# Polochon-street/bliss-rs

Measured on AMD Instinct MI355X. Metric: songs/sec (3-min 22 050 Hz f32) at 1/2/4/8 GPU; HBM GB/s vs roofline, higher is better.
Workload: dtype f32; 1 GPU; configs[1]: batch of 1024 synthetic 3969000-sample (3-min) white-noise f32 PCM buffers per GPU, full 23-feature descriptor set (FeaturesVersion 2); songs_per_gpu=1024, songs_total=1024, features=23, parallelism=single GPU

## Files before the change

bliss-rs_amd/csrc/ctx.hpp:

```cpp
#pragma once
#include <hip/hip_runtime.h>
#include <sched.h>

#include <map>
#include <memory>
#include <mutex>
#include <string>
#include <vector>

#include "../../include/blissgpu.h"
#include "internal.hpp"
#include "resample.hpp"
#include "staging_ring.hpp"

namespace bg {

int fail(int code, const char* what, const char* detail);

#define HIP_TRY(expr)                                                                           \
    do {                                                                                        \
        hipError_t e_ = (expr);                                                                 \
        if (e_ != hipSuccess) return ::bg::fail(BLISSGPU_ERR_HIP, #expr, hipGetErrorString(e_)); \
    } while (0)

struct EventPair { hipEvent_t a, b; };

template <typename T>
struct DevBuf {
    T* p = nullptr;
    size_t cap = 0;
    int ensure(size_t n) {
        if (n <= cap) return BLISSGPU_OK;
        if (p) (void)hipFree(p);
        p = nullptr;
        cap = 0;
        size_t want = n + n / 8 + 64;
        hipError_t e = hipMalloc((void**)&p, want * sizeof(T));
        if (e != hipSuccess && want > n) {
            (void)hipGetLastError();
            want = n;
            e = hipMalloc((void**)&p, want * sizeof(T));
        }
        if (e != hipSuccess) {
            (void)hipGetLastError();
            p = nullptr;
            return fail(BLISSGPU_ERR_OOM, "hipMalloc", hipGetErrorString(e));
        }
        cap = want;
        return BLISSGPU_OK;
    }
    void release() { if (p) (void)hipFree(p); p = nullptr; cap = 0; }
};

template <typename T>
struct PinnedBuf {
    T* p = nullptr;
    size_t cap = 0;
    int ensure(size_t n) {
        if (n <= cap) return BLISSGPU_OK;
        if (p) (void)hipHostFree(p);
        p = nullptr;
        cap = 0;
        const size_t want = n + n / 4 + 64;
        hipError_t e = hipHostMalloc((void**)&p, want * sizeof(T), hipHostMallocDefault);
        if (e != hipSuccess) { (void)hipGetLastError(); p = nullptr; return fail(BLISSGPU_ERR_OOM, "hipHostMalloc", hipGetErrorString(e)); }
        cap = want;
        return BLISSGPU_OK;
    }
    void release() { if (p) (void)hipHostFree(p); p = nullptr; cap = 0; }
};

struct ChunkSlot {
    DevBuf<uint8_t> slab;
    DevBuf<uint8_t> desc;
    PinnedBuf<uint8_t> h_desc;
    hipEvent_t ev_start = nullptr, ev_fork = nullptr, ev_stft = nullptr, ev_sel = nullptr, ev_tune = nullptr, ev_sum = nullptr, ev_chroma = nullptr;
    hipEvent_t ev_acf = nullptr, ev_beat = nullptr;
    bool beat_masked = false;
    static constexpr int MAX_PIECES = 8;
    hipEvent_t ev_piece[MAX_PIECES] = {};
    int pieces = 0;
    bg::SongRange piece[MAX_PIECES]{};
    hipEvent_t ev_desc = nullptr;
    hipEvent_t ev_free = nullptr;
    bool used = false;
    bool back_pending = false;
    Batch batch{};
    Workspace ws{};
};

#ifndef FEED_COPY_STREAMS
#define FEED_COPY_STREAMS 2
#endif
#ifndef STAGE_LANES_DEFAULT
#define STAGE_LANES_DEFAULT 4
#endif
#ifndef STAGE_SLABS_DEFAULT
#define STAGE_SLABS_DEFAULT 3
#endif
#ifndef STAGE_SLAB_KIB_DEFAULT
#define STAGE_SLAB_KIB_DEFAULT 4096
#endif
#ifndef STAGE_EVENT_FLAGS
#define STAGE_EVENT_FLAGS (hipEventDisableTiming | hipEventBlockingSync)
#endif
constexpr int N_COPY_STREAMS = FEED_COPY_STREAMS;
#ifndef FEED_BUFFERS
#define FEED_BUFFERS 3
#endif
constexpr int N_FEED_BUFFERS = FEED_BUFFERS;
constexpr uint32_t MAX_SAMPLE_RATE = 768000;
struct FeedSong {
    const void* p;
    uint64_t frames;
    uint32_t rate;
    uint8_t fmt;
    uint8_t channels;
    size_t frame_bytes() const { return (size_t)(fmt == BLISSGPU_SAMPLE_S16 ? 2 : 4) * channels; }
    bool direct() const { return fmt == BLISSGPU_SAMPLE_F32 && channels == 1 && rate == SWR_OUT_RATE; }
};
struct ResampleBank {
    SwrPlan plan;
    float* d_bank = nullptr;
    size_t bytes = 0;
    uint64_t last_use = 0;
};
#ifndef SWR_CACHE_BYTES
#define SWR_CACHE_BYTES (64ull << 20)
#endif

constexpr int MAX_STAGE_LANES = 16;
struct HipStageDev {
    int device;
    hipStream_t* streams;
    std::vector<int> cpus;
    void thread_begin(int) {
        (void)hipSetDevice(device);
        if (!cpus.empty()) {
            cpu_set_t set;
            CPU_ZERO(&set);
            for (int cpu : cpus)
                if (cpu >= 0 && cpu < CPU_SETSIZE) CPU_SET(cpu, &set);
            (void)sched_setaffinity(0, sizeof(set), &set);
        }
    }
    void* slab_alloc(size_t bytes) {
        void* p = nullptr;
        if (hipHostMalloc(&p, bytes, hipHostMallocDefault) != hipSuccess) { (void)hipGetLastError(); return nullptr; }
        return p;
    }
    void slab_free(void* p) { (void)hipHostFree(p); }
    void* event_create() {
        hipEvent_t e = nullptr;
        if (hipEventCreateWithFlags(&e, STAGE_EVENT_FLAGS) != hipSuccess) { (void)hipGetLastError(); return nullptr; }
        return (void*)e;
    }
    void event_destroy(void* e) { (void)hipEventDestroy((hipEvent_t)e); }
    int copy_async(void* dst, const void* slab, size_t bytes, int lane) {
        return (int)hipMemcpyAsync(dst, slab, bytes, hipMemcpyHostToDevice, streams[lane]);
    }
    int event_record(void* ev, int lane) { return (int)hipEventRecord((hipEvent_t)ev, streams[lane]); }
    int event_wait(void* ev) { return (int)hipEventSynchronize((hipEvent_t)ev); }
    std::string error_string(int code) { return hipGetErrorString((hipError_t)code); }
};

struct HostFeed {
    DevBuf<float> pcm[N_FEED_BUFFERS];
    DevBuf<uint8_t> raw[N_FEED_BUFFERS];
    DevBuf<float> out[N_FEED_BUFFERS];
    hipEvent_t ev_copied[N_FEED_BUFFERS][N_COPY_STREAMS] = {}, ev_done[N_FEED_BUFFERS] = {};
    hipStream_t copy_stream[N_COPY_STREAMS] = {};
    StageConfig stage_cfg{STAGE_LANES_DEFAULT, STAGE_SLABS_DEFAULT, (size_t)STAGE_SLAB_KIB_DEFAULT << 10};
    std::unique_ptr<StagingRing<HipStageDev>> ring;
    hipStream_t lane_stream[MAX_STAGE_LANES] = {};
    hipEvent_t ev_lane[N_FEED_BUFFERS][MAX_STAGE_LANES] = {};
    bool stage_numa = false;
    bool stage_numa_known = false;
    uint64_t staged_calls = 0;
    uint64_t staged_bytes = 0;
};

}

struct blissgpu_ctx {
    int device = 0;
    std::recursive_mutex mu;
    hipStream_t own_stream = nullptr;
    hipStream_t stream = nullptr;
    hipStream_t aux_stream = nullptr;
    hipStream_t chr_stream = nullptr;
    hipStream_t mask_stream = nullptr;
    int mask_cus = 0;
    int tail_mode = -1;
    uint32_t pipeline_chunks = 1;
    hipEvent_t ev_interop = nullptr;
    bool rolloff_exact_all = false;
    bool flux_order = false;
    int stft_shape = 0;
    int tail_split = 0;
    bool debug_chroma = false;
    bool serial = false;
    bool counted_live = false;
    uint64_t ws_limit = 0;
    uint32_t cand_budget = bg::CAND_BUDGET_PER_FRAME;
    float2 *tw8192 = nullptr, *tw512 = nullptr;
    float *hann8192 = nullptr, *hannz512 = nullptr, *bt_rwv = nullptr, *bt_dfwv = nullptr;
    double* chroma_bank = nullptr;
    bg::DeviceTables tables{};
    bg::ChunkSlot slot[2];
    uint64_t chunk_seq = 0;
    bg::DevBuf<int32_t> dbg_tuning;
    bg::DevBuf<uint32_t> dbg_nbpms;
    bg::DevBuf<double> dbg_chroma, dbg_interval;
    uint32_t dbg_n = 0;
    bg::Workspace last_ws{};
    std::vector<bg::SongDesc> last_songs;
    uint64_t last_chunks = 0;
    bg::HostFeed feed;
    std::map<uint32_t, bg::ResampleBank> swr_banks;
    size_t swr_bytes = 0;
    uint64_t swr_clock = 0;
    int64_t forest_split = 0;
    bool forest_global = false;
    int64_t forest_group_nodes = 0;
    bg::DevBuf<uint32_t> gf_img[2];
    bg::PinnedBuf<uint32_t> gf_host[2];
    hipEvent_t gf_ev[2] = {nullptr, nullptr};
    double gf_build_ms = 0.0, gf_wait_ms = 0.0;
    uint64_t gf_batches = 0;
    int n_cus = 0;
    bg::DevBuf<uint32_t> pl_sync, pl_keys;
    bg::DevBuf<uint32_t> pl_next;
    bg::DevBuf<uint8_t> pl_tmp;
    bg::DevBuf<unsigned long long> pl_slots;
    bg::DevBuf<uint8_t> pl_chain;
    bg::DevBuf<uint8_t> km_ws;
    uint64_t km_loop_copies = 0, km_loop_bytes = 0;
// ... 76 lines not shown
```

bliss-rs_amd/csrc/kernels_tempo.hip:

```cpp
#include "device_utils.hpp"
#include "internal.hpp"

namespace bg {

__device__ __forceinline__ float exp_f32(float x) { return (float)exp((double)x); }

__global__ __launch_bounds__(256) void onset_kernel(const SongDesc* __restrict__ songs,
                                                    const float* __restrict__ flux,
                                                    float* __restrict__ thresholded) {
    const SongDesc sd = songs[blockIdx.y];
    const uint32_t t = blockIdx.x * 256 + threadIdx.x;
    if (!sd.ok || t >= sd.n_b) return;
    const float* f = flux + sd.b_off;
    float p[7], tmp[7];
#pragma unroll
    for (int i = 0; i < 7; i++) {
        const long idx = (long)t - 6 + i;
        p[i] = idx >= 0 ? f[idx] : 0.0f;
    }
    const float b0 = 0.1599879f, b1 = 0.31997577f, b2 = 0.1599879f, a1 = 0.23484048f, a2 = 0.0f;
    float x1 = 0.f, x2 = 0.f, y1 = 0.f, y2 = 0.f;
#pragma unroll
    for (int i = 0; i < 7; i++) {
        const float x0 = p[i];
        const float y0 = b0 * x0 + b1 * x1 + b2 * x2 - a1 * y1 - a2 * y2;
        x2 = x1; x1 = x0; y2 = y1; y1 = y0;
        p[i] = y0;
    }
#pragma unroll
    for (int i = 0; i < 7; i++) tmp[6 - i] = p[i];
    x1 = x2 = y1 = y2 = 0.f;
#pragma unroll
    for (int i = 0; i < 7; i++) {
        const float x0 = tmp[i];
        const float y0 = b0 * x0 + b1 * x1 + b2 * x2 - a1 * y1 - a2 * y2;
        x2 = x1; x1 = x0; y2 = y1; y1 = y0;
        tmp[i] = y0;
    }
#pragma unroll
    for (int i = 0; i < 7; i++) p[i] = tmp[6 - i];
    float sum = 0.0f;
#pragma unroll
    for (int i = 0; i < 7; i++) sum += p[i];
    const float mean = sum / 7.0f;
    const float p5 = p[5];
#pragma unroll
    for (int i = 0; i < 7; i++)
#pragma unroll
        for (int j = 0; j + 1 < 7 - i; j++) {
            const float lo = fminf(p[j], p[j + 1]), hi = fmaxf(p[j], p[j + 1]);
            p[j] = lo; p[j + 1] = hi;
        }
    const float median = p[3];
    thresholded[sd.b_off + t] = p5 - median - mean * 0.3f;
}

void launch_onset(const Batch& b, const Workspace& w, hipStream_t st) {
    if (b.n_songs == 0 || b.total_b == 0) return;
    hipLaunchKernelGGL(onset_kernel, dim3((uint32_t)((b.max_nb + 255) / 256), b.n_songs), dim3(256), 0, st, b.songs,
                       w.flux, w.thresholded);
}

template <int Q>
__device__ __forceinline__ void wave_argmax_last(const float (&x)[Q], float* val, int* idx) {
    const int lane = lane_id();
    float best = -1.0f;
    int bidx = 0;
#pragma unroll
    for (int q = 0; q < Q; q++) {
        if (x[q] >= 0.0f && x[q] >= best) { best = x[q]; bidx = lane + 64 * q; }
    }
#pragma unroll
    for (int off = 32; off > 0; off >>= 1) {
        const float ov = __shfl_xor(best, off, WAVE);
        const int oi = __shfl_xor(bidx, off, WAVE);
        if (ov > best || (ov == best && oi > bidx)) { best = ov; bidx = oi; }
    }
    *val = best;
    *idx = (best < 0.0f) ? 0 : bidx;
}

__device__ __forceinline__ float quad_peak_pos(const float* x, int len, int pos) {
    if (pos == 0 || pos >= len - 1) return (float)pos;
    const float s0 = x[pos - 1], s1 = x[pos], s2 = x[pos + 1];
    return (float)pos + 0.5f * (s0 - s2) / (s0 - 2.0f * s1 + s2);
}

__device__ float bt_timesig(const float* acf, long gp) {
    if (gp < 2) return 4;
    float three = 0.0f, four = 0.0f;
    const long acflen = BT_WINLEN;
    if (acflen > 6 * gp + 2) {
        for (long k = -2; k < 2; k++) { three += acf[3 * gp + k]; four += acf[4 * gp + k]; }
    } else {
        for (long k = -2; k < 2; k++) {
            const long i3 = 3 * gp + k, i6 = 6 * gp + k, i4 = 4 * gp + k, i2 = 2 * gp + k;
            if (i3 < acflen && i6 < acflen) three += acf[i3] + acf[i6];
            else if (i3 < acflen) three += acf[i3];
            if (i4 < acflen && i2 < acflen) four += acf[i4] + acf[i2];
            else if (i4 < acflen) four += acf[i4];
        }
    }
    return three > four ? 3 : 4;
}

constexpr int BT_PRE_G3 = 0, BT_PRE_G4 = BT_LAGLEN, BT_PRE_RP3 = 256, BT_PRE_RP4 = 257, BT_PRE_TS3 = 258, BT_PRE_TS4 = 259;
static_assert(BT_PRE_STRIDE >= 260, "per-run record");

typedef float bt_f2 __attribute__((ext_vector_type(2)));

constexpr int ACF_RUNS = 8, ACF_PITCH = 580;
static_assert(ACF_PITCH >= BT_WINLEN + 65 && ACF_PITCH % 4 == 0, "zero padding behind a frame, 16-byte aligned frames");

__device__ __forceinline__ void acf_block16(bt_f2 (&acc)[4], const float* w, const float* w1, const float* f) {
    float r[24], r1[24], fv[16];
#pragma unroll
    for (int u = 0; u < 24; u++) { r[u] = w[u]; r1[u] = w1[u]; }
#pragma unroll
    for (int u = 0; u < 16; u++) fv[u] = f[u];
#pragma unroll
    for (int u = 0; u < 16; u += 2) {
        const bt_f2 fv0 = {fv[u], fv[u]}, fv1 = {fv[u + 1], fv[u + 1]};
#pragma unroll
        for (int k = 0; k < 4; k++) {
            const bt_f2 e = {r[u + 2 * k], r[u + 2 * k + 1]};
            acc[k] = acc[k] + fv0 * e;
        }
#pragma unroll
        for (int k = 0; k < 4; k++) {
            const bt_f2 o = {r1[u + 2 * k], r1[u + 2 * k + 1]};
            acc[k] = acc[k] + fv1 * o;
        }
    }
}

__global__ __launch_bounds__(256) void beat_acf_kernel(const SongDesc* __restrict__ songs,
                                                       const float* __restrict__ thresholded,
                                                       const float* __restrict__ rwv_tab,
                                                       float* __restrict__ pre_all) {
    __shared__ __attribute__((aligned(16))) float df[ACF_RUNS * ACF_PITCH];
    __shared__ __attribute__((aligned(16))) float df1[ACF_RUNS * ACF_PITCH];
    static_assert(ACF_PITCH >= BT_WINLEN && ACF_PITCH >= 2 * BT_LAGLEN, "acf / acfout live in a run's own frame");
    const uint32_t s = blockIdx.y;
    const long m0 = (long)blockIdx.x * ACF_RUNS;
    const SongDesc sd = songs[s];
    if (!sd.ok) return;
    const long n_b = sd.n_b;
    const long n_runs = (n_b >= BT_STEP) ? (n_b - BT_STEP) / BT_STEP + 1 : 0;
    if (m0 >= n_runs) return;
    const int tid = threadIdx.x, lane = tid & 63;
    const int wave = __builtin_amdgcn_readfirstlane(tid >> 6);
    const float* thr = thresholded + sd.b_off;

    {
        constexpr int per = ACF_RUNS * ACF_PITCH / 256 + 1;
        float v[per];
#pragma unroll
        for (int q = 0; q < per; q++) {
            const int e = tid + 256 * q, r = e / ACF_PITCH, i = e - r * ACF_PITCH;
            const long m = m0 + r, xi = 128 * (m + 1) - 512 + i;
            const bool live = e < ACF_RUNS * ACF_PITCH && i < BT_WINLEN && m < n_runs && xi > 0;
            const float x = thr[live ? xi - 1 : 0];
            v[q] = live ? x : 0.0f;
        }
#pragma unroll
        for (int q = 0; q < per; q++) {
            const int e = tid + 256 * q, r = e / ACF_PITCH, i = e - r * ACF_PITCH;
            if (e < ACF_RUNS * ACF_PITCH) {
                df[e] = v[q];
                if (i > 0) df1[e - 1] = v[q];
                if (i == ACF_PITCH - 1) df1[e] = 0.0f;
            }
        }
    }
    __syncthreads();
    const int r = lane >> 3, g = lane & 7;
    const int la = 64 * wave + 8 * g, lb = BT_WINLEN - 8 - 64 * wave - 8 * g;
    bt_f2 sa[4], sb[4];
    {
        const int na = BT_WINLEN - 64 * wave, nb = 64 * (wave + 1);
        const float* fr = df + r * ACF_PITCH;
        const float* fr1 = df1 + r * ACF_PITCH;
#pragma unroll
        for (int k = 0; k < 4; k++) { sa[k] = bt_f2{0.0f, 0.0f}; sb[k] = bt_f2{0.0f, 0.0f}; }
        for (int i = 0; i < na; i += 16) acf_block16(sa, fr + la + i, fr1 + la + i, fr + i);
        for (int i = 0; i < nb; i += 16) acf_block16(sb, fr + lb + i, fr1 + lb + i, fr + i);
    }
    __syncthreads();
    {
        float* acf = df + r * ACF_PITCH;
#pragma unroll
        for (int k = 0; k < 4; k++) {
            acf[la + 2 * k] = sa[k].x / (float)(BT_WINLEN - la - 2 * k);
            acf[la + 2 * k + 1] = sa[k].y / (float)(BT_WINLEN - la - 2 * k - 1);
            acf[lb + 2 * k] = sb[k].x / (float)(BT_WINLEN - lb - 2 * k);
            acf[lb + 2 * k + 1] = sb[k].y / (float)(BT_WINLEN - lb - 2 * k - 1);
        }
    }
    __syncthreads();
    for (int rr = 2 * wave; rr < 2 * wave + 2; rr++) {
        const long m = m0 + rr;
        if (m >= n_runs) break;
        const float* acf = df + rr * ACF_PITCH;
        float* acfout = df1 + rr * ACF_PITCH;
        float* pre = pre_all + ((size_t)(sd.b_off / BT_STEP) + s + (size_t)m) * BT_PRE_STRIDE;
#pragma unroll
        for (int half = 0; half < 2; half++) {
            const int l = lane + 64 * half;
            float v3 = 0.0f, v4 = 0.0f, g3 = 0.0f, g4 = 0.0f;
            if (l >= 1 && l < BT_LAGLEN - 1) {
                float v = 0.0f, gs = 0.0f;
                for (int a = 1; a <= 4; a++) {
                    if (a == 4) { v3 = v; g3 = gs; }
                    for (int b = 1; b < 2 * a; b++) {
                        const int idx = l * a + b - 1;
                        if (idx < BT_WINLEN) {
                            v += acf[idx] / (2.0f * (float)a - 1.0f);
                            gs += acf[idx];
                        }
                    }
                }
                v4 = v; g4 = gs;
            }
            const float rw = rwv_tab[l];
            acfout[l] = v3 * rw;
            acfout[BT_LAGLEN + l] = v4 * rw;
            pre[BT_PRE_G3 + l] = g3;
            pre[BT_PRE_G4 + l] = g4;
        }
        __builtin_amdgcn_fence(__ATOMIC_RELEASE, "wavefront");
        __builtin_amdgcn_wave_barrier();
        __builtin_amdgcn_fence(__ATOMIC_ACQUIRE, "wavefront");
#pragma unroll
        for (int which = 0; which < 2; which++) {
            const float* ao = acfout + which * BT_LAGLEN;
            const float x[2] = {ao[lane], ao[lane + 64]};
            float best;
            int maxindex;
            wave_argmax_last(x, &best, &maxindex);
            if (lane == 0) {
                const int rayparam = 43;
                const float rp = (maxindex > 0 && maxindex < BT_LAGLEN - 1) ? quad_peak_pos(ao, BT_LAGLEN, maxindex)
                                                                           : (float)rayparam;
                pre[BT_PRE_RP3 + which] = rp;
                pre[BT_PRE_TS3 + which] = bt_timesig(acf, (long)rp);
            }
        }
    }
}

struct BtShared {
    float dfrev[BT_WINLEN];
    float acfout[BT_LAGLEN];
    float phout[BT_LAGLEN + 1];
    float out[BT_STEP];
};

__global__ __launch_bounds__(64) void beat_track_kernel(const SongDesc* __restrict__ songs,
                                                        const float* __restrict__ thresholded,
                                                        const float* __restrict__ e256,
                                                        const float* __restrict__ dfwv_tab,
                                                        const float* __restrict__ pre_all,
                                                        float* __restrict__ run_bpm, uint32_t* __restrict__ run_cnt,
                                                        uint32_t runs_pitch, TempoState* __restrict__ tempo_out) {
    __shared__ BtShared sh;
    const uint32_t s = blockIdx.x;
    const SongDesc sd = songs[s];
    const int lane = threadIdx.x;
    if (!sd.ok) {
        if (lane == 0) { tempo_out[s].tempo = -1.0f; tempo_out[s].n_bpms = 0; }
        return;
    }
    const float* thr = thresholded + sd.b_off;
    const float* en = e256 + sd.e_off;
    const float* pre_song = pre_all + ((size_t)(sd.b_off / BT_STEP) + s) * BT_PRE_STRIDE;
    float* rbpm = run_bpm + (size_t)s * runs_pitch;
    uint32_t* rcnt = run_cnt + (size_t)s * runs_pitch;

    float dfwv[8];
#pragma unroll
    for (int q = 0; q < 8; q++) dfwv[q] = dfwv_tab[lane + 64 * q];
    float gwv[2] = {0.0f, 0.0f};
    if (lane == 0) sh.phout[BT_LAGLEN] = 0.0f;
    float gp_state = 0.0f, rp1 = 0.0f, rp2 = 0.0f, lastbeat = 0.0f;
    int counter = 0, flagstep = 0, timesig = 0;

    const float g_var = 3.901f;
    const long n_b = sd.n_b;
    long n_runs = (n_b >= BT_STEP) ? (n_b - BT_STEP) / BT_STEP + 1 : 0;
    if (n_runs > (long)runs_pitch) n_runs = (long)runs_pitch;

    struct RunIn {
        float f[8];
        float g3[2], g4[2];
        float rp3, rp4, ts3, ts4;
        float e[2], e1[2];
    };
    auto fetch = [&](long m, RunIn& r) {
#pragma unroll
        for (int q = 0; q < 8; q++) {
            const long xi = 128 * (m + 1) - 512 + lane + 64 * q;
            r.f[q] = (xi <= 0) ? 0.0f : thr[xi - 1];
        }
        const float* pre = pre_song + (size_t)m * BT_PRE_STRIDE;
#pragma unroll
        for (int q = 0; q < 2; q++) {
            r.g3[q] = pre[BT_PRE_G3 + lane + 64 * q];
            r.g4[q] = pre[BT_PRE_G4 + lane + 64 * q];
            const long t = 127 + 128 * m + lane + 64 * q;
            r.e[q] = t < n_b ? en[t] : 1.0f;
            r.e1[q] = t < n_b ? en[t + 1] : 1.0f;
        }
        r.rp3 = pre[BT_PRE_RP3]; r.rp4 = pre[BT_PRE_RP4]; r.ts3 = pre[BT_PRE_TS3]; r.ts4 = pre[BT_PRE_TS4];
    };
    RunIn cur, nxt;
    if (n_runs > 0) fetch(0, cur);

    for (long m = 0; m < n_runs; m++) {
        if (m + 1 < n_runs) fetch(m + 1, nxt);
#pragma unroll
        for (int q = 0; q < 8; q++) sh.dfrev[BT_WINLEN - 1 - (lane + 64 * q)] = cur.f[q] * dfwv[q];
        const float rp = (timesig == 3) ? cur.rp3 : cur.rp4;

        float gp = gp_state;
        if (gp > 0.0f) {
            const float x[2] = {(timesig == 3 ? cur.g3[0] : cur.g4[0]) * gwv[0], (timesig == 3 ? cur.g3[1] : cur.g4[1]) * gwv[1]};
            sh.acfout[lane] = x[0];
            sh.acfout[lane + 64] = x[1];
            float best;
            int maxindex;
            wave_argmax_last(x, &best, &maxindex);
            __syncthreads();
            gp = quad_peak_pos(sh.acfout, BT_LAGLEN, maxindex);
        } else {
            gp = 0.0f;
        }
        int flagconst = 0;
        if (counter == 0) {
            if (fabsf(gp - rp) > 2.0f * g_var) { flagstep = 1; counter = 3; }
            else flagstep = 0;
        }
        if (counter == 1 && flagstep == 1) {
            if (fabsf(2.0f * rp - rp1 - rp2) < g_var) { flagconst = 1; counter = 0; }
            else { flagconst = 0; counter = 2; }
        } else if (counter > 0) {
            counter -= 1;
        }
        rp2 = rp1;
        rp1 = rp;
        float bp;
        int phw_mode;
        if (flagconst) {
            gp = rp;
            timesig = (int)((timesig == 3) ? cur.ts3 : cur.ts4);
            bp = gp;
            phw_mode = 0;
        } else if (timesig > 0) {
            bp = gp;
            phw_mode = ((float)BT_STEP > lastbeat) ? 1 : 0;
        } else {
            bp = rp;
            phw_mode = 0;
        }
        const float bpw = bp;
        while (bp > 0.0f && bp < 25.0f) bp *= 2.0f;
        gp_state = gp;
        if (flagconst) {
#pragma unroll
            for (int q = 0; q < 2; q++) {
                const float diff = (float)(lane + 64 * q + 1) - gp;
                gwv[q] = exp_f32(-0.5f * diff * diff / (g_var * g_var));
            }
        }

        uint32_t nbeats = 0;
// ... 133 lines not shown
```

bliss-rs_amd/csrc/scheduler.hip:

```cpp
#include <string.h>

#include <algorithm>
#include <chrono>
#include <condition_variable>
#include <numeric>

#include "coalescing_front.hpp"
#include "ctx.hpp"

using namespace bg;

namespace {

inline size_t align_up(size_t x, size_t a) { return (x + a - 1) / a * a; }

void fill_counts(SongDesc& d) {
    const uint64_t n = d.n;
    d.n_t = (uint32_t)((n - W512) / HOP_T + 1);
    d.n_b = (uint32_t)((n - W512) / HOP_B + 1);
    d.n_f = std::max(d.n_t, 2u * d.n_b);
    d.n_c = (uint32_t)ceilf((float)n / (float)HOP_C);
    d.n_e = (uint32_t)((n + 255) / 256);
    d.n_l = (uint32_t)((n + LOUD_W - 1) / LOUD_W);
}

size_t song_ws_bytes(const SongDesc& d) {
    if (!d.ok) return 256;
    size_t b = 0;
    b += (size_t)d.n_t * 12 + (size_t)d.n_b * 8 + (size_t)d.n_e * 8;
    b += (size_t)d.n_c * (CBINS_PAD * 4 + 4);
    b += (size_t)H1_BINS * 4 + N_TUNING * 4 + sizeof(TuningState) + sizeof(TempoState);
    b += (size_t)d.n_c * CAND_BUDGET_PER_FRAME * 9;
    b += (size_t)d.n_c * (PIP_MAX_PER_FRAME * 4 + 4);
    b += ((size_t)d.n_c / CH_TILE + 1) * 80;
    b += ((size_t)d.n_b / BT_STEP + 2) * (8 + BT_PRE_STRIDE * 4);
    return b + 4096;
}

struct Carver {
    uint8_t* base;
    size_t off = 0;
    template <typename T>
    T* take(size_t n) {
        off = align_up(off, 256);
        T* p = reinterpret_cast<T*>(base + off);
        off += n * sizeof(T);
        return p;
    }
};

struct ChunkTotals {
    uint64_t tot_t = 0, tot_b = 0, tot_c = 0, tot_e = 0;
    uint32_t max_nb = 0, max_nt = 0, max_runs = 1;
    uint32_t tiles_ct = 0;
    uint64_t cand_cap = 0;
};

Workspace carve(uint8_t* base, uint32_t ns, const ChunkTotals& t, size_t* bytes) {
    Carver m{base};
    Workspace w{};
    w.centroid = m.take<float>(t.tot_t); w.rolloff = m.take<float>(t.tot_t); w.flatness = m.take<float>(t.tot_t);
    w.flux = m.take<float>(t.tot_b); w.thresholded = m.take<float>(t.tot_b);
    w.e256 = m.take<float>(t.tot_e); w.zc256 = m.take<uint32_t>(t.tot_e);
    static_assert((size_t)(CBINS_PAD + PIP_MAX_PER_FRAME) * 4 * HOP_T >= (size_t)256 * 4 * HOP_C,
                  "the borrowed stretch must hold one 256-word entry per timbral frame: bytes per chroma frame x samples per "
                  "timbral frame >= bytes per entry x samples per chroma frame");
    w.spec = m.take<float>(t.tot_c * CBINS_PAD + 64);
    w.peak_rec = m.take<uint32_t>(t.tot_c * PIP_MAX_PER_FRAME);
    w.roll_fix_bytes = (size_t)(reinterpret_cast<uint8_t*>(w.peak_rec + t.tot_c * PIP_MAX_PER_FRAME) - reinterpret_cast<uint8_t*>(w.spec));
    w.frame_max = m.take<float>(t.tot_c);
    w.roll_fix = m.take<RollFix>(1);
    w.h1 = m.take<uint32_t>((size_t)ns * H1_BINS); w.hist100 = m.take<uint32_t>((size_t)ns * N_TUNING);
    w.tuning = m.take<TuningState>(ns);
    w.peak_cnt = m.take<uint32_t>(t.tot_c);
    w.cand_mag = m.take<double>(t.cand_cap); w.cand_pb = m.take<uint8_t>(t.cand_cap);
    w.cand_cursor = m.take<uint32_t>(4);
    w.cand_cap = (uint32_t)t.cand_cap;
    w.chroma_part = m.take<double>((size_t)t.tiles_ct * 10 + 16);
    w.tempo = m.take<TempoState>(ns);
    w.run_bpm = m.take<float>((size_t)ns * t.max_runs); w.run_cnt = m.take<uint32_t>((size_t)ns * t.max_runs);
    w.runs_pitch = t.max_runs;
    w.bt_pre = m.take<float>((size_t)(t.tot_b / BT_STEP + ns + 1) * BT_PRE_STRIDE);
    w.summary = m.take<float>((size_t)ns * 16);
    *bytes = m.off + 4096;
    return w;
}

int ensure_mask_stream(blissgpu_ctx* c, int cus) {
    cus = std::max(1, std::min(cus, c->n_cus));
    if (c->mask_stream && c->mask_cus == cus) return BLISSGPU_OK;
    if (c->mask_stream) { (void)hipStreamSynchronize(c->mask_stream); (void)hipStreamDestroy(c->mask_stream); c->mask_stream = nullptr; }
    std::vector<uint32_t> mask((size_t)(c->n_cus + 31) / 32, 0u);
    for (int i = 0; i < cus; i++) mask[(size_t)i / 32] |= 1u << (i % 32);
    HIP_TRY(hipExtStreamCreateWithCUMask(&c->mask_stream, (uint32_t)mask.size(), mask.data()));
    c->mask_cus = cus;
    return BLISSGPU_OK;
}

int ensure_slot_events(ChunkSlot& s) {
    if (s.ev_free) return BLISSGPU_OK;
    hipEvent_t* evs[] = {&s.ev_start, &s.ev_fork, &s.ev_stft, &s.ev_sel, &s.ev_tune, &s.ev_sum, &s.ev_chroma, &s.ev_desc, &s.ev_free, &s.ev_acf, &s.ev_beat};
    for (hipEvent_t* e : evs) HIP_TRY(hipEventCreateWithFlags(e, hipEventDisableTiming));
    for (hipEvent_t& e : s.ev_piece) HIP_TRY(hipEventCreateWithFlags(&e, hipEventDisableTiming));
    return BLISSGPU_OK;
}

int chunk_front(blissgpu_ctx* c, ChunkSlot& slot, const float* d_pcm, SongDesc* songs, uint32_t ns, bool only_chunk) {
    int rc = ensure_slot_events(slot);
    if (rc) return rc;
    std::vector<uint32_t> pfx_f(ns + 1, 0), pfx_c(ns + 1, 0), pfx_ct(ns + 1, 0), pfx_cw(ns + 1, 0);
    ChunkTotals t;
    for (uint32_t i = 0; i < ns; i++) {
        SongDesc& d = songs[i];
        d.t_off = t.tot_t; d.b_off = t.tot_b; d.c_off = t.tot_c; d.e_off = t.tot_e;
        if (d.ok) {
            t.tot_t += d.n_t; t.tot_b += d.n_b; t.tot_c += d.n_c; t.tot_e += d.n_e;
            t.max_nb = std::max(t.max_nb, d.n_b);
            t.max_nt = std::max(t.max_nt, d.n_t);
            t.max_runs = std::max(t.max_runs, d.n_b / BT_STEP + 1);
        }
        pfx_f[i + 1] = pfx_f[i] + (d.ok ? (d.n_f + F512_TILE - 1) / F512_TILE : 0);
        pfx_c[i + 1] = pfx_c[i] + (d.ok ? 4 * ((d.n_c + 4 * STFT_TILE - 1) / (4 * STFT_TILE)) : 0);
        pfx_ct[i + 1] = pfx_ct[i] + (d.ok ? (d.n_c + CH_TILE - 1) / CH_TILE : 0);
        pfx_cw[i + 1] = pfx_cw[i] + (d.ok ? (d.n_c + 4 * CH_TILE - 1) / (4 * CH_TILE) : 0);
    }
    t.tiles_ct = pfx_ct[ns];
    t.cand_cap = std::min<uint64_t>(t.tot_c * (uint64_t)c->cand_budget, 0xFFFFFF00ull) + 64;

    const size_t desc_bytes = align_up(ns * sizeof(SongDesc), 256) + 4 * align_up((ns + 1) * 4, 256) + 256;
    size_t need = 0;
    (void)carve(nullptr, ns, t, &need);
    if ((rc = slot.desc.ensure(desc_bytes))) return rc;
    if ((rc = slot.slab.ensure(need))) return rc;
    if (slot.used) HIP_TRY(hipEventSynchronize(slot.ev_desc));
    if ((rc = slot.h_desc.ensure(desc_bytes))) return rc;

    hipStream_t st = c->stream, sb = c->serial ? c->stream : c->aux_stream, sc = c->serial ? c->stream : c->chr_stream;
    const bool multi = !c->serial;
    if (slot.used && multi) HIP_TRY(hipStreamWaitEvent(st, slot.ev_free, 0));

    uint8_t* h = slot.h_desc.p;
    size_t o = 0;
    const size_t o_songs = o; memcpy(h + o, songs, ns * sizeof(SongDesc)); o = align_up(o + ns * sizeof(SongDesc), 256);
    const size_t o_f = o; memcpy(h + o, pfx_f.data(), (ns + 1) * 4); o = align_up(o + (ns + 1) * 4, 256);
    const size_t o_c = o; memcpy(h + o, pfx_c.data(), (ns + 1) * 4); o = align_up(o + (ns + 1) * 4, 256);
    const size_t o_ct = o; memcpy(h + o, pfx_ct.data(), (ns + 1) * 4); o = align_up(o + (ns + 1) * 4, 256);
    const size_t o_cw = o; memcpy(h + o, pfx_cw.data(), (ns + 1) * 4); o = align_up(o + (ns + 1) * 4, 256);
    HIP_TRY(hipMemcpyAsync(slot.desc.p, h, o, hipMemcpyHostToDevice, st));
    slot.used = true;

    Batch& b = slot.batch;
    b = Batch{};
    b.pcm = d_pcm;
    b.songs = reinterpret_cast<const SongDesc*>(slot.desc.p + o_songs);
    b.n_songs = ns;
    b.pfx_f = reinterpret_cast<const uint32_t*>(slot.desc.p + o_f);
    b.pfx_c = reinterpret_cast<const uint32_t*>(slot.desc.p + o_c);
    b.pfx_ct = reinterpret_cast<const uint32_t*>(slot.desc.p + o_ct);
    b.pfx_cw = reinterpret_cast<const uint32_t*>(slot.desc.p + o_cw);
    b.tiles_f = pfx_f[ns]; b.tiles_c = pfx_c[ns]; b.tiles_ct = pfx_ct[ns]; b.tiles_cw = pfx_cw[ns];
    b.total_b = t.tot_b; b.max_nb = t.max_nb; b.max_nt = t.max_nt;

    size_t used_bytes = 0;
    slot.ws = carve(slot.slab.p, ns, t, &used_bytes);
    slot.ws.dbg_chroma = nullptr;
    slot.ws.dbg_interval = nullptr;
    if (c->debug_chroma) {
        if ((rc = c->dbg_chroma.ensure((size_t)t.tot_c * 12 + 12))) return rc;
        if ((rc = c->dbg_interval.ensure((size_t)ns * 10))) return rc;
        slot.ws.dbg_chroma = c->dbg_chroma.p;
        slot.ws.dbg_interval = c->dbg_interval.p;
    }
    const Workspace& w = slot.ws;
    c->last_ws = w;
    c->last_songs.assign(songs, songs + ns);
    {
        RollFix rf{};
        if ((uint64_t)w.roll_fix_bytes / (256 * 4) < t.tot_t)
            return fail(BLISSGPU_ERR_INVALID, "chunk_front", "internal: the borrowed stretch cannot hold one exact-rolloff entry per timbral frame");
        rf.cap = (uint32_t)t.tot_t;
        rf.mags = w.spec;
        memcpy(h + o, &rf, sizeof(rf));
        HIP_TRY(hipMemcpyAsync(w.roll_fix, h + o, sizeof(rf), hipMemcpyHostToDevice, st));
    }
    HIP_TRY(hipEventRecord(slot.ev_desc, st));

    HIP_TRY(hipMemsetAsync(w.h1, 0, (size_t)ns * H1_BINS * 4, st));
    HIP_TRY(hipMemsetAsync(w.hist100, 0, (size_t)ns * N_TUNING * 4, st));
    HIP_TRY(hipMemsetAsync(w.cand_cursor, 0, 16, st));
    { Prof p(c, K_FFT512); launch_fft512(b, w, c->tables, st, c->rolloff_exact_all, c->flux_order); }
    { Prof p(c, K_ROLLFIX); launch_rolloff_fix(b, w, t.tot_t, st); }
    if (multi) {
        HIP_TRY(hipEventRecord(slot.ev_fork, st));
        HIP_TRY(hipStreamWaitEvent(sb, slot.ev_fork, 0));
    }
    { Prof p(c, K_ONSET, sb); launch_onset(b, w, sb); }
    { Prof p(c, K_SUMMARY, sb); launch_summary(b, w, sb); }
    slot.beat_masked = multi && c->tail_mode >= 2;
    if (slot.beat_masked) {
        if ((rc = ensure_mask_stream(c, c->tail_mode))) return rc;
        { Prof p(c, K_BEAT, sb); launch_beat_acf(b, w, c->tables, sb); }
        HIP_TRY(hipEventRecord(slot.ev_acf, sb));
        HIP_TRY(hipStreamWaitEvent(c->mask_stream, slot.ev_acf, 0));
        { Prof p(c, K_BEAT, c->mask_stream); launch_beat_track(b, w, c->tables, c->mask_stream); }
        HIP_TRY(hipEventRecord(slot.ev_beat, c->mask_stream));
    }
    const bool acf_early = multi && c->tail_mode == -2;
    if (acf_early) { Prof p(c, K_BEAT, sb); launch_beat_acf(b, w, c->tables, sb); }
    const bool beat_last = multi && c->tail_mode == -3;
    const bool beat_late = !slot.beat_masked && !beat_last && (c->tail_mode == 1 || acf_early || (c->tail_mode < 0 && only_chunk));
    if (!beat_late && !slot.beat_masked && !beat_last) { Prof p(c, K_BEAT, sb); launch_beat(b, w, c->tables, sb); }
    { Prof p(c, K_STFT8192); launch_stft8192(b, w, c->tables, st, c->stft_shape); }
    if (multi) {
        HIP_TRY(hipEventRecord(slot.ev_stft, st));
        HIP_TRY(hipStreamWaitEvent(sc, slot.ev_stft, 0));
    }
    slot.pieces = 0;
    if (multi && only_chunk && c->tail_split > 1 && ns >= 2) {
        const int want = std::min<int>(std::min<int>(c->tail_split, ChunkSlot::MAX_PIECES), (int)ns);
        uint32_t s0 = 0;
        for (int k = 0; k < want && s0 < ns; k++) {
            uint32_t s1 = s0 + 1;
            const uint64_t goal = (uint64_t)pfx_ct[ns] * (uint64_t)(k + 1) / (uint64_t)want;
            while (s1 < ns && (k == want - 1 || pfx_ct[s1] < goal)) s1++;
            slot.piece[slot.pieces++] = SongRange{s0, s1, pfx_ct[s0], pfx_ct[s1], pfx_cw[s0], pfx_cw[s1]};
            s0 = s1;
        }
        if (slot.pieces < 2) slot.pieces = 0;
    }
    if (slot.pieces) {
        for (int k = 0; k < slot.pieces; k++) {
            { Prof p(c, K_TUNE_SELECT, sc); launch_tune_select(b, w, sc, &slot.piece[k]); }
            if (k == 1 && beat_late) {
                HIP_TRY(hipEventRecord(slot.ev_sel, sc));
                HIP_TRY(hipStreamWaitEvent(sb, slot.ev_sel, 0));
                Prof p(c, K_BEAT, sb);
                if (acf_early) launch_beat_track(b, w, c->tables, sb); else launch_beat(b, w, c->tables, sb);
            }
            { Prof p(c, K_TUNE_PASS2, sc); launch_tune_pass2(b, w, sc, &slot.piece[k]); }
            { Prof p(c, K_TUNE_FINAL, sc); launch_tune_final(b, w, sc, &slot.piece[k]); }
            HIP_TRY(hipEventRecord(slot.ev_piece[k], sc));
        }
        if (beat_last) {
            HIP_TRY(hipStreamWaitEvent(sb, slot.ev_piece[slot.pieces - 1], 0));
            Prof p(c, K_BEAT, sb);
            launch_beat(b, w, c->tables, sb);
        }
        HIP_TRY(hipGetLastError());
        slot.back_pending = true;
        return BLISSGPU_OK;
    }
    { Prof p(c, K_TUNE_SELECT, sc); launch_tune_select(b, w, sc); }
    if (beat_late) {
        if (multi) {
            HIP_TRY(hipEventRecord(slot.ev_sel, sc));
            HIP_TRY(hipStreamWaitEvent(sb, slot.ev_sel, 0));
        }
        Prof p(c, K_BEAT, sb);
        if (acf_early) launch_beat_track(b, w, c->tables, sb); else launch_beat(b, w, c->tables, sb);
    }
    { Prof p(c, K_TUNE_PASS2, sc); launch_tune_pass2(b, w, sc); }
    { Prof p(c, K_TUNE_FINAL, sc); launch_tune_final(b, w, sc); }
    if (multi) HIP_TRY(hipEventRecord(slot.ev_tune, sc));
    if (beat_last) {
        HIP_TRY(hipStreamWaitEvent(sb, slot.ev_tune, 0));
        Prof p(c, K_BEAT, sb);
        launch_beat(b, w, c->tables, sb);
    }
    HIP_TRY(hipGetLastError());
    slot.back_pending = true;
    return BLISSGPU_OK;
}

int chunk_back(blissgpu_ctx* c, ChunkSlot& slot, uint32_t features_version, float* d_out, int32_t* d_status) {
    if (!slot.back_pending) return BLISSGPU_OK;
    slot.back_pending = false;
    hipStream_t st = c->stream, sb = c->serial ? c->stream : c->aux_stream;
    const bool multi = !c->serial;
    if (slot.pieces) {
        for (int k = 0; k < slot.pieces; k++) {
            HIP_TRY(hipStreamWaitEvent(st, slot.ev_piece[k], 0));
            Prof p(c, K_CHROMA);
            launch_chroma(slot.batch, slot.ws, c->tables, st, &slot.piece[k]);
        }
    } else {
        if (multi) HIP_TRY(hipStreamWaitEvent(st, slot.ev_tune, 0));
        Prof p(c, K_CHROMA);
        launch_chroma(slot.batch, slot.ws, c->tables, st);
    }
    if (multi) {
        HIP_TRY(hipEventRecord(slot.ev_chroma, st));
        HIP_TRY(hipStreamWaitEvent(sb, slot.ev_chroma, 0));
        if (slot.beat_masked) HIP_TRY(hipStreamWaitEvent(sb, slot.ev_beat, 0));
    }
    { Prof p(c, K_FINALIZE, sb); launch_finalize(slot.batch, slot.ws, features_version, d_out, d_status, c->dbg_tuning.p, c->dbg_nbpms.p, sb); }
    if (multi) HIP_TRY(hipEventRecord(slot.ev_free, sb));
    HIP_TRY(hipGetLastError());
    return BLISSGPU_OK;
}

}

namespace bg {

void scheduler_release(blissgpu_ctx* c) {
    for (ChunkSlot& s : c->slot) {
        s.slab.release(); s.desc.release(); s.h_desc.release();
        hipEvent_t evs[] = {s.ev_start, s.ev_fork, s.ev_stft, s.ev_sel, s.ev_tune, s.ev_sum, s.ev_chroma, s.ev_desc, s.ev_free, s.ev_acf, s.ev_beat};
        for (hipEvent_t e : evs)
            if (e) (void)hipEventDestroy(e);
        for (hipEvent_t e : s.ev_piece)
            if (e) (void)hipEventDestroy(e);
        s = ChunkSlot{};
    }
    HostFeed& f = c->feed;
    f.ring.reset();
    for (hipStream_t& ls : f.lane_stream)
        if (ls) { (void)hipStreamSynchronize(ls); (void)hipStreamDestroy(ls); ls = nullptr; }
    for (auto& row : f.ev_lane)
        for (hipEvent_t& ev : row)
            if (ev) { (void)hipEventDestroy(ev); ev = nullptr; }
    for (auto& kv : c->swr_banks)
        if (kv.second.d_bank) (void)hipFree(kv.second.d_bank);
    c->swr_banks.clear();
    c->swr_bytes = 0;
    for (hipStream_t& cs : f.copy_stream)
        if (cs) { (void)hipStreamSynchronize(cs); (void)hipStreamDestroy(cs); cs = nullptr; }
    for (int b = 0; b < N_FEED_BUFFERS; b++) {
        f.pcm[b].release(); f.raw[b].release(); f.out[b].release();
        for (hipEvent_t& ev : f.ev_copied[b])
            if (ev) { (void)hipEventDestroy(ev); ev = nullptr; }
        if (f.ev_done[b]) (void)hipEventDestroy(f.ev_done[b]);
        f.ev_done[b] = nullptr;
    }
}

#ifndef FEED_GROUP_MIB
#define FEED_GROUP_MIB 512
#endif
#ifndef FEED_GROUP_PCM_FACTOR
#define FEED_GROUP_PCM_FACTOR 1
#endif
#ifndef STAGE_MIN_BYTES
#define STAGE_MIN_BYTES (8ull << 20)
#endif
int resample_bank(blissgpu_ctx* c, uint32_t rate, const ResampleBank** out, const char* who) {
    auto it = c->swr_banks.find(rate);
    if (it == c->swr_banks.end()) {
        ResampleBank rb;
        if (rate > MAX_SAMPLE_RATE || !swr_make_plan(rate, &rb.plan))
            return fail(BLISSGPU_ERR_INVALID, who, "sample_rate must be 1 .. 768000 Hz");
        std::vector<float> bank;
        swr_make_filter(rb.plan, bank);
        rb.bytes = bank.size() * sizeof(float);
        while (!c->swr_banks.empty() && c->swr_bytes + rb.bytes > (size_t)SWR_CACHE_BYTES) {
            auto lru = c->swr_banks.begin();
            for (auto q = c->swr_banks.begin(); q != c->swr_banks.end(); ++q)
                if (q->second.last_use < lru->second.last_use) lru = q;
            if (lru->second.d_bank) (void)hipFree(lru->second.d_bank);
            c->swr_bytes -= lru->second.bytes;
            c->swr_banks.erase(lru);
        }
        float* d = nullptr;
        hipError_t e = hipMalloc((void**)&d, rb.bytes);
        if (e != hipSuccess) { (void)hipGetLastError(); return fail(BLISSGPU_ERR_OOM, "hipMalloc(resample bank)", hipGetErrorString(e)); }
        e = hipMemcpy(d, bank.data(), rb.bytes, hipMemcpyHostToDevice);
        if (e != hipSuccess) { (void)hipFree(d); return fail(BLISSGPU_ERR_HIP, "hipMemcpy(resample bank)", hipGetErrorString(e)); }
        rb.d_bank = d;
        c->swr_bytes += rb.bytes;
        it = c->swr_banks.emplace(rate, rb).first;
    }
    it->second.last_use = ++c->swr_clock;
    *out = &it->second;
    return BLISSGPU_OK;
}

std::vector<int> parse_cpulist(const char* text) {
    std::vector<int> cpus;
    for (const char* p = text; p && *p;) {
        char* end = nullptr;
        const long a = strtol(p, &end, 10);
        if (end == p || a < 0) break;
        long b = a;
        if (*end == '-') {
            const char* q = end + 1;
            b = strtol(q, &end, 10);
            if (end == q || b < a) break;
        }
        for (long v = a; v <= b && cpus.size() < 4096; v++) cpus.push_back((int)v);
        p = *end == ',' ? end + 1 : end;
        if (*end != ',') break;
    }
    return cpus;
}

std::vector<int> device_local_cpus(int device) {
    char bus[32] = {0};
    if (hipDeviceGetPCIBusId(bus, (int)sizeof(bus), device) != hipSuccess) { (void)hipGetLastError(); return {}; }
    for (char* p = bus; *p; p++) *p = (char)tolower((unsigned char)*p);
    const std::string base = std::string("/sys/bus/pci/devices/") + bus;
    char line[4096] = {0};
    int node = -1;
    if (FILE* f = fopen((base + "/numa_node").c_str(), "r")) {
        if (fgets(line, sizeof(line), f)) node = atoi(line);
        fclose(f);
    }
    if (node < 0) return {};
    std::vector<int> cpus;
    if (FILE* f = fopen((base + "/local_cpulist").c_str(), "r")) {
        if (fgets(line, sizeof(line), f)) cpus = parse_cpulist(line);
        fclose(f);
    }
    return cpus;
}

int enqueue_decode(blissgpu_ctx* c, const void* d_in, int fmt, uint32_t channels, uint64_t frames, uint32_t rate, float* d_out,
                   uint64_t n_out, hipStream_t st, const char* who) {
    if (rate == SWR_OUT_RATE) {
        launch_pcm_convert(d_in, fmt, channels, d_out, frames, st);
        HIP_TRY(hipGetLastError());
        return BLISSGPU_OK;
    }
    const ResampleBank* rb;
    const int rc = resample_bank(c, rate, &rb, who);
    if (rc) return rc;
    HIP_TRY(launch_resample(d_in, fmt, channels, frames, rb->plan, rb->d_bank, d_out, n_out, st));
    return BLISSGPU_OK;
}

int analyze_host_songs(blissgpu_ctx* c, const FeedSong* in, uint32_t n_songs, uint32_t features_version, float* out,
                       int32_t* status, const char* who, float* d_rows) {
    const uint32_t d = blissgpu_feature_count(features_version);
    if (!d) return fail(BLISSGPU_ERR_INVALID, who, "features_version must be 1 or 2");
    if (n_songs == 0) return BLISSGPU_OK;
    std::vector<uint64_t> out_len(n_songs);
    bool any_raw = false;
    for (uint32_t i = 0; i < n_songs; i++) {
        const FeedSong& fs = in[i];
        if (fs.channels == 0 || fs.channels > 8) return fail(BLISSGPU_ERR_INVALID, who, "channels must be 1..8");
        if (fs.fmt != BLISSGPU_SAMPLE_F32 && fs.fmt != BLISSGPU_SAMPLE_S16 && fs.fmt != BLISSGPU_SAMPLE_S32)
            return fail(BLISSGPU_ERR_INVALID, who, "sample_format must be F32, S16 or S32");
        if (fs.rate == 0 || fs.rate > MAX_SAMPLE_RATE) return fail(BLISSGPU_ERR_INVALID, who, "sample_rate must be 1 .. 768000 Hz");
        if (fs.frames && !fs.p) return fail(BLISSGPU_ERR_INVALID, who, "NULL song pointer");
        if (fs.rate == SWR_OUT_RATE) out_len[i] = fs.frames;
        else {
            SwrPlan pl;
            swr_make_plan(fs.rate, &pl);
            out_len[i] = swr_out_len(pl, fs.frames);
        }
        any_raw = any_raw || !fs.direct();
    }
    std::lock_guard<std::recursive_mutex> lk(c->mu);
    HIP_TRY(hipSetDevice(c->device));
    HostFeed& f = c->feed;
    {
        uint32_t last_rate = SWR_OUT_RATE;
        for (uint32_t i = 0; i < n_songs; i++)
            if (in[i].rate != SWR_OUT_RATE && in[i].rate != last_rate && in[i].frames) {
                const ResampleBank* rb;
                const int brc = resample_bank(c, in[i].rate, &rb, who);
                if (brc) return brc;
// ... 532 lines not shown
```

Before: 28200 songs/sec.

## Replace ACF divisions with exact reciprocal-FMA and reschedule rolloff/finalize streams

Adds an exact-division helper that swaps float divides for a reciprocal multiply plus an FMA correction, with a wave-uniform range check that falls back to true division. It is used in the beat ACF normalisation and the comb-sum loops. Separately, the rolloff fix kernel now launches after the stream fork so onset can overlap it, and for single-chunk runs finalize moves onto the main stream, waiting on a tail event instead of bouncing through the aux stream. The aim is to cut divide latency and cross-stream serialisation, at the cost of extra events and branch code.

Measured after the change: 28310 songs/sec, median of 6. About the same (+0.4%).

```diff
diff --git a/bliss-rs_amd/csrc/ctx.hpp b/bliss-rs_amd/csrc/ctx.hpp
--- a/bliss-rs_amd/csrc/ctx.hpp
+++ b/bliss-rs_amd/csrc/ctx.hpp
@@ -83,6 +83,9 @@
     bg::SongRange piece[MAX_PIECES]{};
     hipEvent_t ev_desc = nullptr;
     hipEvent_t ev_free = nullptr;
+    hipEvent_t ev_roll = nullptr;
+    hipEvent_t ev_tail = nullptr;
+    bool assemble_main = false;
     bool used = false;
     bool back_pending = false;
     Batch batch{};
diff --git a/bliss-rs_amd/csrc/exact_div.hpp b/bliss-rs_amd/csrc/exact_div.hpp
--- /dev/null
+++ b/bliss-rs_amd/csrc/exact_div.hpp
@@ -0,0 +1,48 @@
+#pragma once
+#include <math.h>
+
+#if defined(__HIPCC__) || defined(__CUDACC__)
+#define EXACT_DIV_HD __host__ __device__ __forceinline__
+#else
+#define EXACT_DIV_HD inline
+#endif
+
+namespace bg {
+
+constexpr float EXACT_DIV_MIN = 0x1p-60f;
+constexpr float EXACT_DIV_MAX = 3.40282347e+38f;
+constexpr int EXACT_DIV_TABLE = 512;
+
+EXACT_DIV_HD bool exact_div_ok(float x) {
+    const float a = fabsf(x);
+    return a >= EXACT_DIV_MIN && a <= EXACT_DIV_MAX;
+}
+
+EXACT_DIV_HD float exact_div_fast(float x, float c, float y) {
+    const float q = x * y;
+    const float r = fmaf(-c, q, x);
+    return fmaf(r, y, q);
+}
+
+EXACT_DIV_HD float exact_div(float x, float c, float y) { return exact_div_ok(x) ? exact_div_fast(x, c, y) : x / c; }
+
+template <int C>
+EXACT_DIV_HD float exact_div_fast(float x) {
+    static_assert(C >= 1 && C <= EXACT_DIV_TABLE, "proved for 1 .. 512 only");
+    if (C == 1) return x;
+    return exact_div_fast(x, (float)C, 1.0f / (float)C);
+}
+template <int C>
+EXACT_DIV_HD float exact_div(float x) {
+    if (C == 1) return x;
+    return exact_div_ok(x) ? exact_div_fast<C>(x) : x / (float)C;
+}
+
+struct ExactDivRecip {
+    float y[EXACT_DIV_TABLE + 1];
+    constexpr ExactDivRecip() : y() {
+        for (int c = 1; c <= EXACT_DIV_TABLE; c++) y[c] = 1.0f / (float)c;
+    }
+};
+
+}
diff --git a/bliss-rs_amd/csrc/kernels_tempo.hip b/bliss-rs_amd/csrc/kernels_tempo.hip
--- a/bliss-rs_amd/csrc/kernels_tempo.hip
+++ b/bliss-rs_amd/csrc/kernels_tempo.hip
@@ -1,4 +1,5 @@
 #include "device_utils.hpp"
+#include "exact_div.hpp"
 #include "internal.hpp"
 
 namespace bg {
@@ -132,6 +133,32 @@
             acc[k] = acc[k] + fv1 * o;
         }
     }
+}
+
+__device__ const ExactDivRecip acf_recip = ExactDivRecip();
+__device__ __forceinline__ bool acf_div_ok(float x) { return exact_div_ok(x) || __float_as_uint(x) == 0u; }
+
+template <bool FAST, int A>
+__device__ __forceinline__ void comb_terms(const float* acf, int l, float& v, float& gs) {
+#pragma unroll
+    for (int b = 1; b < 2 * A; b++) {
+        const int idx = l * A + b - 1;
+        if (idx < BT_WINLEN) {
+            const float x = acf[idx];
+            v += FAST ? exact_div_fast<2 * A - 1>(x) : x / (2.0f * (float)A - 1.0f);
+            gs += x;
+        }
+    }
+}
+template <bool FAST>
+__device__ __forceinline__ void comb_sums(const float* acf, int l, float& v3, float& v4, float& g3, float& g4) {
+    float v = 0.0f, gs = 0.0f;
+    comb_terms<FAST, 1>(acf, l, v, gs);
+    comb_terms<FAST, 2>(acf, l, v, gs);
+    comb_terms<FAST, 3>(acf, l, v, gs);
+    v3 = v; g3 = gs;
+    comb_terms<FAST, 4>(acf, l, v, gs);
+    v4 = v; g4 = gs;
 }
 
 __global__ __launch_bounds__(256) void beat_acf_kernel(const SongDesc* __restrict__ songs,
@@ -189,12 +216,37 @@
     __syncthreads();
     {
         float* acf = df + r * ACF_PITCH;
+        float s[16], c[16];
 #pragma unroll
         for (int k = 0; k < 4; k++) {
-            acf[la + 2 * k] = sa[k].x / (float)(BT_WINLEN - la - 2 * k);
-            acf[la + 2 * k + 1] = sa[k].y / (float)(BT_WINLEN - la - 2 * k - 1);
-            acf[lb + 2 * k] = sb[k].x / (float)(BT_WINLEN - lb - 2 * k);
-            acf[lb + 2 * k + 1] = sb[k].y / (float)(BT_WINLEN - lb - 2 * k - 1);
+            s[4 * k] = sa[k].x; c[4 * k] = (float)(BT_WINLEN - la - 2 * k);
+            s[4 * k + 1] = sa[k].y; c[4 * k + 1] = (float)(BT_WINLEN - la - 2 * k - 1);
+            s[4 * k + 2] = sb[k].x; c[4 * k + 2] = (float)(BT_WINLEN - lb - 2 * k);
+            s[4 * k + 3] = sb[k].y; c[4 * k + 3] = (float)(BT_WINLEN - lb - 2 * k - 1);
+        }
+        bool fast = true;
+#pragma unroll
+        for (int u = 0; u < 16; u++) fast = fast && acf_div_ok(s[u]);
+        if (__all(fast)) {
+            const float* ya = acf_recip.y + (BT_WINLEN - la);
+            const float* yb = acf_recip.y + (BT_WINLEN - lb);
+#pragma unroll
+            for (int k = 0; k < 4; k++) {
+                s[4 * k] = exact_div_fast(s[4 * k], c[4 * k], ya[-2 * k]);
+                s[4 * k + 1] = exact_div_fast(s[4 * k + 1], c[4 * k + 1], ya[-2 * k - 1]);
+                s[4 * k + 2] = exact_div_fast(s[4 * k + 2], c[4 * k + 2], yb[-2 * k]);
+                s[4 * k + 3] = exact_div_fast(s[4 * k + 3], c[4 * k + 3], yb[-2 * k - 1]);
+            }
+        } else {
+#pragma unroll
+            for (int u = 0; u < 16; u++) s[u] = s[u] / c[u];
+        }
+#pragma unroll
+        for (int k = 0; k < 4; k++) {
+            acf[la + 2 * k] = s[4 * k];
+            acf[la + 2 * k + 1] = s[4 * k + 1];
+            acf[lb + 2 * k] = s[4 * k + 2];
+            acf[lb + 2 * k + 1] = s[4 * k + 3];
         }
     }
     __syncthreads();
@@ -204,23 +256,17 @@
         const float* acf = df + rr * ACF_PITCH;
         float* acfout = df1 + rr * ACF_PITCH;
         float* pre = pre_all + ((size_t)(sd.b_off / BT_STEP) + s + (size_t)m) * BT_PRE_STRIDE;
+        bool ok = true;
+#pragma unroll
+        for (int q = 0; q < BT_WINLEN / 64; q++) ok = ok && acf_div_ok(acf[lane + 64 * q]);
+        const bool fast = __all(ok);
 #pragma unroll
         for (int half = 0; half < 2; half++) {
             const int l = lane + 64 * half;
             float v3 = 0.0f, v4 = 0.0f, g3 = 0.0f, g4 = 0.0f;
             if (l >= 1 && l < BT_LAGLEN - 1) {
-                float v = 0.0f, gs = 0.0f;
-                for (int a = 1; a <= 4; a++) {
-                    if (a == 4) { v3 = v; g3 = gs; }
-                    for (int b = 1; b < 2 * a; b++) {
-                        const int idx = l * a + b - 1;
-                        if (idx < BT_WINLEN) {
-                            v += acf[idx] / (2.0f * (float)a - 1.0f);
-                            gs += acf[idx];
-                        }
-                    }
-                }
-                v4 = v; g4 = gs;
+                if (fast) comb_sums<true>(acf, l, v3, v4, g3, g4);
+                else comb_sums<false>(acf, l, v3, v4, g3, g4);
             }
             const float rw = rwv_tab[l];
             acfout[l] = v3 * rw;
diff --git a/bliss-rs_amd/csrc/scheduler.hip b/bliss-rs_amd/csrc/scheduler.hip
--- a/bliss-rs_amd/csrc/scheduler.hip
+++ b/bliss-rs_amd/csrc/scheduler.hip
@@ -99,7 +99,7 @@
 
 int ensure_slot_events(ChunkSlot& s) {
     if (s.ev_free) return BLISSGPU_OK;
-    hipEvent_t* evs[] = {&s.ev_start, &s.ev_fork, &s.ev_stft, &s.ev_sel, &s.ev_tune, &s.ev_sum, &s.ev_chroma, &s.ev_desc, &s.ev_free, &s.ev_acf, &s.ev_beat};
+    hipEvent_t* evs[] = {&s.ev_start, &s.ev_fork, &s.ev_stft, &s.ev_sel, &s.ev_tune, &s.ev_sum, &s.ev_chroma, &s.ev_desc, &s.ev_free, &s.ev_acf, &s.ev_beat, &s.ev_roll, &s.ev_tail};
     for (hipEvent_t* e : evs) HIP_TRY(hipEventCreateWithFlags(e, hipEventDisableTiming));
     for (hipEvent_t& e : s.ev_piece) HIP_TRY(hipEventCreateWithFlags(&e, hipEventDisableTiming));
     return BLISSGPU_OK;
@@ -189,14 +189,17 @@
     HIP_TRY(hipMemsetAsync(w.hist100, 0, (size_t)ns * N_TUNING * 4, st));
     HIP_TRY(hipMemsetAsync(w.cand_cursor, 0, 16, st));
     { Prof p(c, K_FFT512); launch_fft512(b, w, c->tables, st, c->rolloff_exact_all, c->flux_order); }
-    { Prof p(c, K_ROLLFIX); launch_rolloff_fix(b, w, t.tot_t, st); }
     if (multi) {
         HIP_TRY(hipEventRecord(slot.ev_fork, st));
         HIP_TRY(hipStreamWaitEvent(sb, slot.ev_fork, 0));
     }
+    { Prof p(c, K_ROLLFIX); launch_rolloff_fix(b, w, t.tot_t, st); }
+    if (multi) HIP_TRY(hipEventRecord(slot.ev_roll, st));
     { Prof p(c, K_ONSET, sb); launch_onset(b, w, sb); }
+    if (multi) HIP_TRY(hipStreamWaitEvent(sb, slot.ev_roll, 0));
     { Prof p(c, K_SUMMARY, sb); launch_summary(b, w, sb); }
     slot.beat_masked = multi && c->tail_mode >= 2;
+    slot.assemble_main = multi && only_chunk;
     if (slot.beat_masked) {
         if ((rc = ensure_mask_stream(c, c->tail_mode))) return rc;
         { Prof p(c, K_BEAT, sb); launch_beat_acf(b, w, c->tables, sb); }
@@ -246,6 +249,7 @@
             Prof p(c, K_BEAT, sb);
             launch_beat(b, w, c->tables, sb);
         }
+        if (slot.assemble_main) HIP_TRY(hipEventRecord(slot.ev_tail, sb));
         HIP_TRY(hipGetLastError());
         slot.back_pending = true;
         return BLISSGPU_OK;
@@ -267,6 +271,7 @@
         Prof p(c, K_BEAT, sb);
         launch_beat(b, w, c->tables, sb);
     }
+    if (slot.assemble_main) HIP_TRY(hipEventRecord(slot.ev_tail, sb));
     HIP_TRY(hipGetLastError());
     slot.back_pending = true;
     return BLISSGPU_OK;
@@ -288,9 +293,14 @@
         Prof p(c, K_CHROMA);
         launch_chroma(slot.batch, slot.ws, c->tables, st);
     }
+    if (slot.assemble_main) sb = st;
     if (multi) {
-        HIP_TRY(hipEventRecord(slot.ev_chroma, st));
-        HIP_TRY(hipStreamWaitEvent(sb, slot.ev_chroma, 0));
+        if (slot.assemble_main) {
+            HIP_TRY(hipStreamWaitEvent(st, slot.ev_tail, 0));
+        } else {
+            HIP_TRY(hipEventRecord(slot.ev_chroma, st));
+            HIP_TRY(hipStreamWaitEvent(sb, slot.ev_chroma, 0));
+        }
         if (slot.beat_masked) HIP_TRY(hipStreamWaitEvent(sb, slot.ev_beat, 0));
     }
     { Prof p(c, K_FINALIZE, sb); launch_finalize(slot.batch, slot.ws, features_version, d_out, d_status, c->dbg_tuning.p, c->dbg_nbpms.p, sb); }
@@ -306,7 +316,7 @@
 void scheduler_release(blissgpu_ctx* c) {
     for (ChunkSlot& s : c->slot) {
         s.slab.release(); s.desc.release(); s.h_desc.release();
-        hipEvent_t evs[] = {s.ev_start, s.ev_fork, s.ev_stft, s.ev_sel, s.ev_tune, s.ev_sum, s.ev_chroma, s.ev_desc, s.ev_free, s.ev_acf, s.ev_beat};
+        hipEvent_t evs[] = {s.ev_start, s.ev_fork, s.ev_stft, s.ev_sel, s.ev_tune, s.ev_sum, s.ev_chroma, s.ev_desc, s.ev_free, s.ev_acf, s.ev_beat, s.ev_roll, s.ev_tail};
         for (hipEvent_t e : evs)
             if (e) (void)hipEventDestroy(e);
         for (hipEvent_t e : s.ev_piece)
```
